# pomelyu/gaussian_splatting_lightning

Measured on AMD Instinct MI355X. Metric: rasterizer fwd+bwd ms & Gaussians·pixels/s @ 1M gauss, 1080p; 1/2/4/8-GPU, higher is better.
Workload: dtype f32; 1 GPU; BASELINE config 3/4: 1M Gaussians, 1920x1080, SH deg 3, fwd+bwd, one view per GPU; gaussians=1000000, width=1920, height=1080, sh_degree=3, parallelism=dp1 (one view per GPU, gradient exchange: none), instances_per_view=4156425, sum_n_contrib=318481376, stage_events=none

## Files before the change

gaussian_splatting_lightning_amd/csrc/gsr_bin.hip:

```cpp
#include <algorithm>

#include "gsr_kernels.h"

namespace gsr {



template <int BKW>
__device__ void bk_instance_offsets(const BucketParams &p, uint32_t g_lo, uint32_t g_hi, uint32_t *s_tmp) {
    const int tid = threadIdx.x, w = tid >> 6, lane = tid & 63;
    uint32_t acc = 0;
    for (uint32_t k = tid; k < g_lo / 256; k += 64 * BKW) acc += p.block_sums[k];
#pragma unroll
    for (int o = 32; o > 0; o >>= 1) acc += (uint32_t)__shfl_xor((int)acc, o);
    if (lane == 0) s_tmp[w] = acc;
    __syncthreads();
    uint32_t base = 0;
    for (int k = 0; k < BKW; k++) base += s_tmp[k];
    __syncthreads();
    for (uint32_t r0 = g_lo; r0 < g_hi; r0 += 4 * 64 * BKW) {
        const uint32_t g = r0 + 4 * (uint32_t)tid;
        uint32_t v[4], loc = 0;
#pragma unroll
        for (int k = 0; k < 4; k++) {
            v[k] = g + k < g_hi ? p.tiles[g + k] : 0u;
            loc += v[k];
        }
        const uint32_t inc = wave_inclusive_scan(loc, lane);
        if (lane == 63) s_tmp[w] = inc;
        __syncthreads();
        uint32_t run = base + inc - loc, all = 0;
        for (int k = 0; k < BKW; k++) {
            if (k < w) run += s_tmp[k];
            all += s_tmp[k];
        }
#pragma unroll
        for (int k = 0; k < 4; k++) {
            if (g + k < g_hi) p.inst_start[g + k] = run;
            run += v[k];
        }
        base += all;
        __syncthreads();
    }
    if (g_hi == p.P && tid == 0) p.inst_start[p.P] = base;
}

__device__ __forceinline__ uint32_t bk_walk_blocks(const BucketParams &p) {
    const uint32_t nbig = *p.nbig;
    return nbig > p.nr ? min(p.nb, nbig) : p.nr;
}

template <bool SCATTER, int BKW>
__global__ __launch_bounds__(64 * BKW) void bk_walk_kernel(BucketParams p) {
    extern __shared__ uint32_t s_tab[];
    __shared__ uint4 s_rec[BKW][64];
    __shared__ uint4 s_aux[BKW][64];
    __shared__ int s_own[BKW][64];
    static_assert(BKW * 64 >= LPT_HIST_WORDS, "the LPT workgroup's histogram lives in s_own");
    const int tid = threadIdx.x, w = tid >> 6, lane = tid & 63;
    const uint32_t b = blockIdx.x, T = p.T, gx = (uint32_t)p.gx;
    if (SCATTER && b == p.nb) {
        constexpr bool xok = 64 * BKW == 1024 && sizeof(s_rec) >= 4 * (LPT_BCNT_WORDS + LPT_XCD + 17);
        lpt_order_block(p.ranges, nullptr, 0, (int)T, p.lpt_shift, p.order, reinterpret_cast<uint32_t *>(&s_own[0][0]),
                        xok ? p.order_xcd : nullptr, reinterpret_cast<uint32_t *>(&s_rec[0][0]), p.gx,
                        (int)((T + gx - 1) / gx), 4);
        return;
    }
    const uint32_t nbw = bk_walk_blocks(p);
    if (b >= nbw) return;
    const bool reg = SCATTER && p.keys_reg != nullptr;
    if (SCATTER && reg) {
        const uint32_t *hrow = p.hist_pre + (size_t)b * T;
        const uint32_t nr = (T + BK_REGION - 1) / BK_REGION;
        for (uint32_t r = tid; r < nr; r += 64 * BKW) {
            const uint32_t t0 = r * BK_REGION;
            uint32_t acc = p.tile_start[t0], v[BK_REGION];
#pragma unroll
            for (int q = 0; q < BK_REGION; q++) v[q] = hrow[min(t0 + q, T - 1)];
#pragma unroll
            for (int q = 0; q < BK_REGION; q++) acc += t0 + q < T ? v[q] : 0u;
            s_tab[r] = acc;
        }
    } else if (SCATTER) {
        const uint32_t *hrow = p.hist_pre + (size_t)b * T;
        for (uint32_t t = tid; t < T; t += 64 * BKW) s_tab[t] = p.tile_start[t] + hrow[t];
    } else {
        for (uint32_t t = tid; t < T; t += 64 * BKW) s_tab[t] = 0u;
    }
    s_own[w][lane] = -1;
    const uint32_t g_lo = min(p.P, b * p.gper), g_hi = min(p.P, g_lo + p.gper);
    if (!SCATTER && b < p.nr) bk_instance_offsets<BKW>(p, g_lo, g_hi, reinterpret_cast<uint32_t *>(&s_aux[0][0]));
    __syncthreads();
    uint32_t g = g_lo + (uint32_t)w * 64 + lane;
    uint32_t n_kept = 0, n_u = 0, n_dep = 0;
    uint4 n_e = make_uint4(0, 0, 0, 0);
    if (g < g_hi) {
        n_kept = p.tiles[g];
        n_e = p.exp_rec[g];
        if (SCATTER) {
            n_u = p.inst_start[g];
            n_dep = p.depth_key[g];
        }
    }
    for (uint32_t g0 = g_lo + (uint32_t)w * 64; g0 < g_hi; g0 += 64 * BKW) {
        const uint32_t kept = n_kept, u = n_u, dep = n_dep;
        const uint4 e = n_e;
        g = g0 + 64 * BKW + lane;
        n_kept = 0;
        if (g < g_hi) {
            n_kept = p.tiles[g];
            n_e = p.exp_rec[g];
            if (SCATTER) {
                n_u = p.inst_start[g];
                n_dep = p.depth_key[g];
            }
        }
        uint32_t len = 0;
        const uint64_t m = (uint64_t)e.x | ((uint64_t)e.y << 32);
        if (kept > 0 && kept <= BIG_GAUSSIAN_TILES) len = m ? 64u - (uint32_t)__builtin_clzll(m) : kept;
        const uint32_t incl = wave_inclusive_scan(len, lane);
        const uint32_t total = (uint32_t)__builtin_amdgcn_readlane((int)incl, 63);
        const uint32_t start = incl - len;
        s_rec[w][lane] = e;
        s_aux[w][lane] = make_uint4(start, u, dep, __float_as_uint(len ? 1.0f / (float)e.w : 0.f));
        int carry = -1;
        for (uint32_t B = 0; B < total; B += 64) {
            const bool marks = len > 0 && start >= B && start < B + 64;
            if (marks) s_own[w][start - B] = lane;
            wave_lds_sync();
            const int o = max(wave_inclusive_max(s_own[w][lane]), carry);
            carry = __builtin_amdgcn_readlane(o, 63);
            wave_lds_sync();
            if (marks) s_own[w][start - B] = -1;
            const uint32_t j = B + (uint32_t)lane;
            if (j < total) {
                const uint4 r = s_rec[w][o];
                const uint4 x = s_aux[w][o];
                const uint32_t c = j - x.x;
                const uint64_t mo = (uint64_t)r.x | ((uint64_t)r.y << 32);
                if (!mo || ((mo >> c) & 1ull)) {
                    const uint32_t tile = rect_tile(c, r.z & 0xffffu, r.z >> 16, r.w, __uint_as_float(x.w), gx);
                    if (!SCATTER) {
                        atomicAdd(&s_tab[tile], 1u);
                    } else {
                        const uint32_t ui = x.y + (mo ? (uint32_t)__popcll(mo & ((1ull << c) - 1ull)) : c);
                        const unsigned long long key = ((unsigned long long)x.z << 32) | ui;
                        if (reg) {
                            const uint32_t slot = atomicAdd(&s_tab[tile / BK_REGION], 1u);
                            p.keys_reg[slot] = key | ((unsigned long long)(tile % BK_REGION) << BK_REG_SHIFT);
                        } else {
                            p.keys[atomicAdd(&s_tab[tile], 1u)] = key;
                        }
                        p.inst_gid[ui] = g0 + (uint32_t)o;
                        p.inv[ui] = INV_NONE;
                    }
                }
            }
        }
        wave_lds_sync();
    }
    const uint32_t nbig = *p.nbig;
    for (uint32_t bi = b; bi < nbig; bi += nbw) {
        const uint32_t gb = p.big_list[bi];
        const uint4 e = p.exp_rec[gb];
        const uint32_t area = p.tiles[gb];
        const float inv_w = 1.0f / (float)e.w;
        const uint32_t u0 = SCATTER ? p.inst_start[gb] : 0u;
        const unsigned long long dk = SCATTER ? ((unsigned long long)p.depth_key[gb] << 32) : 0ull;
        for (uint32_t c = tid; c < area; c += 64 * BKW) {
            const uint32_t tile = rect_tile(c, e.z & 0xffffu, e.z >> 16, e.w, inv_w, gx);
            if (!SCATTER) {
                atomicAdd(&s_tab[tile], 1u);
            } else {
                if (reg) {
                    const uint32_t slot = atomicAdd(&s_tab[tile / BK_REGION], 1u);
                    p.keys_reg[slot] = (dk | (u0 + c)) | ((unsigned long long)(tile % BK_REGION) << BK_REG_SHIFT);
                } else {
                    p.keys[atomicAdd(&s_tab[tile], 1u)] = dk | (u0 + c);
                }
                p.inst_gid[u0 + c] = gb;
                p.inv[u0 + c] = INV_NONE;
            }
        }
    }
    if (!SCATTER) {
        __syncthreads();
        uint32_t *row = p.hist + (size_t)b * T;
        for (uint32_t t = tid; t < T; t += 64 * BKW) row[t] = s_tab[t];
    }
}

__device__ __forceinline__ uint32_t bk_row_block(uint32_t r, uint32_t nb, int xcd_major) {
    if (!xcd_major) return r;
    const uint32_t q = nb >> 3, rem = nb & 7u;
    const uint32_t big = rem * (q + 1);
    uint32_t x, k;
    if (r < big) {
        x = r / (q + 1);
        k = r - x * (q + 1);
    } else {
        const uint32_t r2 = r - big;
        x = rem + r2 / q;
        k = r2 - (x - rem) * q;
    }
    return k * 8 + x;
}

template <int CW, int TW = 64>
__global__ __launch_bounds__(64 * CW) void bk_columns_kernel(BucketParams p) {
    static_assert(TW == 64 || TW == 32, "tiles per workgroup");
    constexpr int NH = 64 / TW;
    __shared__ uint32_t s_sum[CW][64];
    __shared__ uint32_t s_bid;
    __shared__ unsigned long long s_excl;
    const uint32_t *__restrict__ hist = p.hist;
    uint32_t *__restrict__ hist_pre = p.hist_pre;
    const uint32_t nb = bk_walk_blocks(p), T = p.T;
    const int tid = threadIdx.x, w = tid >> 6, lane = tid & 63;
    const int sub = lane % TW, h = lane / TW;
    if (tid == 0) s_bid = atomicAdd(p.ticket, 1u);
    if (blockIdx.x == 0 && p.lpt_bcnt)
        for (uint32_t k = (uint32_t)tid; k < LPT_BCNT_WORDS; k += blockDim.x) p.lpt_bcnt[k] = 0u;
    __syncthreads();
    const uint32_t bid = s_bid;
    const uint32_t t = bid * TW + sub;
    const uint32_t q = (nb + CW - 1) / CW, r0w = min(nb, w * q), r1w = min(nb, r0w + q);
    const uint32_t qh = (q + NH - 1) / NH, r0 = min(r1w, r0w + h * qh), r1 = min(r1w, r0 + qh);
    uint32_t sum = 0;
    const int xm = p.xcd_major;
    if (t < T) {
        uint32_t r = r0;
        for (; r + 8 <= r1; r += 8) {
            uint32_t v[8];
#pragma unroll
            for (int i = 0; i < 8; i++) v[i] = hist[(size_t)bk_row_block(r + i, nb, xm) * T + t];
#pragma unroll
            for (int i = 0; i < 8; i++) sum += v[i];
        }
        for (; r < r1; r++) sum += hist[(size_t)bk_row_block(r, nb, xm) * T + t];
    }
    uint32_t lowsum = 0;
    if constexpr (NH == 2) {
        const uint32_t other = (uint32_t)__shfl_xor((int)sum, 32);
        lowsum = h ? other : 0u;
        sum += other;
    }
    if (h == 0) s_sum[w][sub] = sum;
    __syncthreads();
    uint32_t tot = 0;
#pragma unroll
    for (int i = 0; i < CW; i++) tot += s_sum[i][sub];
    if (w == 0) {
        const uint32_t tv = h == 0 ? tot : 0u;
        const uint32_t inc = wave_inclusive_scan(tv, lane);
        auto agg_of = [&](uint32_t qq) -> uint64_t {
            const uint32_t tq = qq * TW + sub;
            uint64_t v = 0;
            if (tq < T && h == 0)
                for (uint32_t r = 0; r < nb; r++) v += hist[(size_t)r * T + tq];
            return wave_sum_u64(v);
        };
        const uint64_t excl = wave_lookback(p.tile_status, bid, (uint64_t)__builtin_amdgcn_readlane((int)inc, 63),
                                            lane, p.err, p.lb_patience, p.lb_force != 0, agg_of);
        const bool mine = t < T && h == 0;
        if (mine) {
            const uint32_t st = (uint32_t)(excl + inc - tot);
            p.tile_start[t] = st;
            p.ranges[t] = tot ? make_uint2(st, st + tot) : make_uint2(0, 0);
            p.tile_next[t] = st;
            if (t % BK_REGION == 0) p.reg_start[t / BK_REGION] = st;
            p.tile_last[t] = 0u;
            p.tile_loaded[t] = 0u;
            if (t == T - 1) {
                p.tile_start[T] = st + tot;
                p.reg_start[(T + BK_REGION - 1) / BK_REGION] = st + tot;
            }
        }
        const bool l0 = mine && tot > SEG_CAP && tot <= SEG_BLOCK_CAP, l1 = mine && tot > SEG_BLOCK_CAP;
        const uint64_t m0 = __ballot(l0), m1 = __ballot(l1);
        uint32_t b0 = 0, b1 = 0;
        if (lane == 0) {
            if (m0) b0 = atomicAdd(&p.long_cnt[0], (uint32_t)__popcll(m0));
            if (m1) b1 = atomicAdd(&p.long_cnt[1], (uint32_t)__popcll(m1));
        }
        b0 = __builtin_amdgcn_readfirstlane(b0);
        b1 = __builtin_amdgcn_readfirstlane(b1);
        const uint64_t lt = lanemask_lt(lane);
        if (l0) p.long_list[b0 + __popcll(m0 & lt)] = t;
        if (l1) p.long_list[(T + 1) + b1 + __popcll(m1 & lt)] = t;
    }
    uint32_t run = lowsum;
    for (int i = 0; i < w; i++) run += s_sum[i][sub];
    if (t < T) {
        uint32_t r = r0;
        for (; r + 8 <= r1; r += 8) {
            uint32_t v[8];
            size_t row[8];
#pragma unroll
            for (int i = 0; i < 8; i++) {
                row[i] = (size_t)bk_row_block(r + i, nb, xm) * T + t;
                v[i] = hist[row[i]];
            }
#pragma unroll
            for (int i = 0; i < 8; i++) {
                hist_pre[row[i]] = run;
                run += v[i];
            }
        }
        for (; r < r1; r++) {
            const size_t row = (size_t)bk_row_block(r, nb, xm) * T + t;
            const uint32_t v = hist[row];
            hist_pre[row] = run;
            run += v;
        }
    }
}

#ifndef GSR_PART_THREADS
#define GSR_PART_THREADS 256
#endif
#ifndef GSR_PART_ITEMS
#define GSR_PART_ITEMS 4
#endif
constexpr int PART_THREADS = GSR_PART_THREADS;
constexpr int PART_ITEMS = GSR_PART_ITEMS;
constexpr uint32_t PART_CHUNK = PART_THREADS * PART_ITEMS;
#ifndef GSR_PART_MAXR
#define GSR_PART_MAXR 4
#endif
constexpr uint32_t PART_MAXR = GSR_PART_MAXR;
constexpr uint32_t PART_BINS = PART_MAXR * BK_REGION;
static_assert(PART_BINS % 64 == 0 && PART_BINS >= 64, "the bin scan gives each lane of one wave PART_BINS / 64 bins");
__device__ __forceinline__ uint32_t bk_region_of(const uint32_t *rs, uint32_t lo, uint32_t n, uint32_t i) {
    uint32_t hi = n - 1;
    while (lo < hi) {
        const uint32_t mid = (lo + hi + 1) >> 1;
        if (rs[mid] <= i) lo = mid; else hi = mid - 1;
    }
    return lo;
}
__global__ __launch_bounds__(PART_THREADS) void bk_partition_kernel(BucketParams p) {
    __shared__ unsigned long long s_keys[PART_CHUNK];
    __shared__ uint16_t s_bin[PART_CHUNK];
    __shared__ uint32_t s_cnt[PART_BINS], s_lstart[PART_BINS], s_gbase[PART_BINS];
    __shared__ uint32_t s_rstart[PART_MAXR + 1];
    __shared__ uint32_t s_nle[2];
    constexpr unsigned long long TB_MASK = (unsigned long long)(BK_REGION - 1) << BK_REG_SHIFT;
    const uint32_t T = p.T, nr = (T + BK_REGION - 1) / BK_REGION, R = p.tile_start[T];
    const uint32_t c0 = blockIdx.x * PART_CHUNK;
    if (c0 >= R) return;
    const uint32_t n = min(PART_CHUNK, R - c0);
    const int tid = threadIdx.x;
    unsigned long long k[PART_ITEMS];
#pragma unroll
    for (int q = 0; q < PART_ITEMS; q++)
        k[q] = p.keys_reg[c0 + min((uint32_t)(q * PART_THREADS + tid), n - 1)];
    if (tid < 64) {
        const uint32_t rlo = wave_last_le(p.reg_start, nr - 1, c0, tid);
        const uint32_t rhi = wave_last_le(p.reg_start, nr - 1, c0 + n - 1, tid);
        if (tid == 0) {
            s_nle[0] = rlo;
            s_nle[1] = rhi;
        }
    }
    __syncthreads();
    const uint32_t rlo = s_nle[0], nreg = s_nle[1] - rlo + 1;
    if (nreg > PART_MAXR) {
        for (uint32_t i = c0 + tid; i < c0 + n; i += PART_THREADS) {
            const unsigned long long k = p.keys_reg[i];
            const uint32_t t = bk_region_of(p.reg_start, rlo, rlo + nreg, i) * BK_REGION +
                               (uint32_t)((k & TB_MASK) >> BK_REG_SHIFT);
            p.keys[atomicAdd(&p.tile_next[t], 1u)] = k & ~TB_MASK;
        }
        return;
    }
    for (uint32_t j = tid; j <= nreg; j += PART_THREADS) s_rstart[j] = p.reg_start[rlo + j];
    for (uint32_t j = tid; j < nreg * BK_REGION; j += PART_THREADS) s_cnt[j] = 0u;
    __syncthreads();
    uint32_t bin[PART_ITEMS], rank[PART_ITEMS];
#pragma unroll
    for (int q = 0; q < PART_ITEMS; q++) {
        const uint32_t i = (uint32_t)(q * PART_THREADS + tid);
        rank[q] = 0xffffffffu;
        bin[q] = 0;
        if (i < n) {
            uint32_t j = 0;
#pragma unroll
            for (uint32_t step = PART_MAXR / 2; step; step >>= 1)
                if (j + step < nreg && s_rstart[j + step] <= c0 + i) j += step;
            bin[q] = j * BK_REGION + (uint32_t)((k[q] & TB_MASK) >> BK_REG_SHIFT);
            rank[q] = atomicAdd(&s_cnt[bin[q]], 1u);
        }
    }
    __syncthreads();
    const uint32_t nbins = nreg * BK_REGION;
    if (tid < 64) {
        constexpr int PER = PART_BINS / 64;
        uint32_t c[PER], sum = 0;
#pragma unroll
        for (int q = 0; q < PER; q++) {
            const uint32_t b = (uint32_t)(tid * PER + q);
            c[q] = b < nbins ? s_cnt[b] : 0u;
            sum += c[q];
        }
        uint32_t run = wave_inclusive_scan(sum, tid) - sum;
#pragma unroll
        for (int q = 0; q < PER; q++) {
            const uint32_t b = (uint32_t)(tid * PER + q);
            if (b < nbins) {
                s_lstart[b] = run;
                if (c[q]) s_gbase[b] = atomicAdd(&p.tile_next[(rlo + b / BK_REGION) * BK_REGION + b % BK_REGION], c[q]);
            }
            run += c[q];
        }
    }
    __syncthreads();
#pragma unroll
    for (int q = 0; q < PART_ITEMS; q++)
        if (rank[q] != 0xffffffffu) {
            const uint32_t pos = s_lstart[bin[q]] + rank[q];
            s_keys[pos] = k[q] & ~TB_MASK;
            s_bin[pos] = (uint16_t)bin[q];
        }
    __syncthreads();
#pragma unroll
    for (int q = 0; q < PART_ITEMS; q++) {
        const uint32_t i = (uint32_t)(q * PART_THREADS + tid);
        if (i < n) {
            const uint32_t b = s_bin[i];
            p.keys[s_gbase[b] + (i - s_lstart[b])] = s_keys[i];
        }
    }
}

template <int E>
__device__ __forceinline__ void seg_sort_wave32(const unsigned long long *__restrict__ keys, uint32_t start, uint32_t n,
                                                unsigned long long *__restrict__ scratch, int lane,
                                                unsigned long long (&out)[E]) {
    constexpr int LOGE = (E >= 8) ? 3 : (E >= 4) ? 2 : (E >= 2) ? 1 : 0;
    constexpr int IDXB = LOGE + 6;
    const uint32_t base = (uint32_t)lane * E;
    unsigned long long x64[E];
    uint32_t dmin = 0xffffffffu, dmax = 0u;
#pragma unroll
    for (int r = 0; r < E; r++) x64[r] = keys[start + min(base + r, n - 1)];
#pragma unroll
    for (int r = 0; r < E; r++) {
        const bool valid = base + r < n;
        x64[r] = valid ? x64[r] : ~0ull;
        scratch[base + r] = x64[r];
        const uint32_t d = (uint32_t)(x64[r] >> 32);
        if (valid) {
            dmin = min(dmin, d);
            dmax = max(dmax, d);
        }
    }
#pragma unroll
    for (int o = 32; o > 0; o >>= 1) {
        dmin = min(dmin, (uint32_t)__shfl_xor((int)dmin, o));
        dmax = max(dmax, (uint32_t)__shfl_xor((int)dmax, o));
    }
    const uint32_t range = dmax - dmin;
    const int bits = range ? 32 - __builtin_clz(range) : 0;
    const int sh = bits > 32 - IDXB ? bits - (32 - IDXB) : 0;
    uint32_t x[E];
#pragma unroll
    for (int r = 0; r < E; r++)
        x[r] = (base + r < n) ? ((((uint32_t)(x64[r] >> 32) - dmin) >> sh) << IDXB) | (base + r) : 0xffffffffu;
#pragma unroll
    for (int lk = 1; lk < LOGE; lk++) {
#pragma unroll
        for (int lj = lk - 1; lj >= 0; lj--) {
#pragma unroll
            for (int r = 0; r < E; r++) {
                if (r & (1 << lj)) continue;
                const uint32_t a = x[r], c = x[r | (1 << lj)];
                const uint32_t lo = min(a, c), hi = max(a, c);
                const bool asc = (r & (1 << lk)) == 0;
                x[r] = asc ? lo : hi;
                x[r | (1 << lj)] = asc ? hi : lo;
            }
        }
    }
    for (int lk = LOGE > 1 ? LOGE : 1; lk <= LOGE + 6; lk++) {
        const uint32_t flip = (base & (1u << lk)) ? 0xffffffffu : 0u;
#pragma unroll
        for (int r = 0; r < E; r++) x[r] ^= flip;
        for (int lj = lk - 1; lj >= LOGE; lj--) {
            const int lm = 1 << (lj - LOGE);
            const bool lower = (lane & lm) == 0;
            const int addr = (lane ^ lm) << 2;
            uint32_t y[E];
#pragma unroll
            for (int r = 0; r < E; r++) y[r] = (uint32_t)__builtin_amdgcn_ds_bpermute(addr, (int)x[r]);
#pragma unroll
            for (int r = 0; r < E; r++) x[r] = lower ? min(x[r], y[r]) : max(x[r], y[r]);
        }
#pragma unroll
        for (int lj = LOGE - 1; lj >= 0; lj--) {
#pragma unroll
            for (int r = 0; r < E; r++) {
                if (r & (1 << lj)) continue;
                const uint32_t a = x[r], c = x[r | (1 << lj)];
                x[r] = min(a, c);
                x[r | (1 << lj)] = max(a, c);
            }
        }
#pragma unroll
        for (int r = 0; r < E; r++) x[r] ^= flip;
    }
    const uint32_t next0 = (uint32_t)__shfl_down((int)x[0], 1);
    bool tie = false;
#pragma unroll
    for (int r = 0; r < E; r++) {
        const uint32_t nx = r + 1 < E ? x[r + 1] : next0;
        const bool both = base + r + 1 < n && (r + 1 < E || lane < 63);
        tie |= both && (x[r] >> IDXB) == (nx >> IDXB);
    }
    const bool any_tie = __ballot(tie) != 0;
    wave_lds_sync();
#pragma unroll
    for (int r = 0; r < E; r++) out[r] = scratch[x[r] & ((1u << IDXB) - 1u)];
    if (!any_tie) return;
    for (uint32_t it = 0; it < n; it++) {
        bool sw = false;
        auto ce = [&](unsigned long long &a, unsigned long long &b) {
            const bool s = b < a;
            const unsigned long long lo = s ? b : a, hi = s ? a : b;
            a = lo;
            b = hi;
            sw |= s;
        };
        if (E == 1) {
            const unsigned long long y = __shfl_xor(out[0], 1);
            const bool lower = (lane & 1) == 0;
            const unsigned long long v = lower ? (y < out[0] ? y : out[0]) : (y > out[0] ? y : out[0]);
            sw |= v != out[0];
            out[0] = v;
        } else {
#pragma unroll
            for (int r = 0; r + 1 < E; r += 2) ce(out[r], out[r + 1]);
        }
#pragma unroll
        for (int r = 1; r + 1 < E; r += 2) ce(out[r], out[r + 1]);
        const unsigned long long nx = __shfl_down(out[0], 1), pv = __shfl_up(out[E - 1], 1);
        const bool low_end = E > 1 || (lane & 1), high_end = E > 1 || !(lane & 1);
        if (low_end && lane < 63 && nx < out[E - 1]) {
            out[E - 1] = nx;
            sw = true;
        }
        if (high_end && lane > 0 && out[0] < pv) {
            out[0] = pv;
            sw = true;
        }
        if (!__ballot(sw)) return;
    }
}

template <int E>
__device__ __forceinline__ void seg_sort_wave(const unsigned long long *keys, uint32_t start, uint32_t n,
                                              uint32_t *sorted_u, int lane, unsigned long long *scratch) {
    unsigned long long y[E];
    seg_sort_wave32<E>(keys, start, n, scratch, lane, y);
    const uint32_t base = (uint32_t)lane * E;
#pragma unroll
    for (int r = 0; r < E; r++)
        if (base + r < n) sorted_u[start + base + r] = (uint32_t)y[r];
}
template <int E>
__device__ __forceinline__ void seg_sort_wave_to_lds(const unsigned long long *keys, uint32_t start, uint32_t n,
                                                     unsigned long long *lds_out, int lane) {
    unsigned long long y[E];
    seg_sort_wave32<E>(keys, start, n, lds_out, lane, y);
    wave_lds_sync();
    const uint32_t base = (uint32_t)lane * E;
#pragma unroll
    for (int r = 0; r < E; r++) lds_out[base + r] = y[r];
}

constexpr uint32_t SB_CHUNK = 512;
constexpr uint32_t SB_WAVE_SCRATCH = SEG_BLOCK_CAP / 4;

template <int PER>
__device__ __forceinline__ void seg_merge_ranks(const unsigned long long *__restrict__ s_x, uint32_t n, uint32_t nch,
                                                uint32_t start, uint32_t *__restrict__ sorted_u,
                                                unsigned long long *__restrict__ keys_out) {
    const uint32_t span = nch * SB_CHUNK;
    for (uint32_t e0 = 0; e0 < n; e0 += 256 * PER) {
        unsigned long long key[PER];
        uint32_t pos[PER], own[PER];
#pragma unroll
        for (int i = 0; i < PER; i++) {
            const uint32_t e = e0 + threadIdx.x + 256u * i;
            key[i] = e < n ? s_x[e] : ~0ull;
            pos[i] = e & (SB_CHUNK - 1);
            own[i] = e < n ? (e & ~(SB_CHUNK - 1)) : 0u;
        }
        for (uint32_t d = SB_CHUNK; d < span; d += SB_CHUNK) {
            uint32_t lo[PER], idx[PER];
#pragma unroll
            for (int i = 0; i < PER; i++) {
                lo[i] = own[i] + d;
                if (lo[i] >= span) lo[i] -= span;
                idx[i] = lo[i];
            }
#pragma unroll
            for (uint32_t step = SB_CHUNK / 2; step; step >>= 1) {
#pragma unroll
                for (int i = 0; i < PER; i++)
                    if (s_x[idx[i] + step - 1] < key[i]) idx[i] += step;
            }
#pragma unroll
            for (int i = 0; i < PER; i++)
                pos[i] += idx[i] - lo[i] + (s_x[idx[i]] < key[i] ? 1u : 0u);
        }
#pragma unroll
        for (int i = 0; i < PER; i++) {
            const uint32_t e = e0 + threadIdx.x + 256u * i;
            if (e >= n) continue;
            if (keys_out) keys_out[start + pos[i]] = key[i];
            else sorted_u[start + pos[i]] = (uint32_t)key[i];
        }
    }
}

__device__ __forceinline__ void seg_lds_sort(const unsigned long long *__restrict__ keys, uint32_t start, uint32_t n,
                                             uint32_t *__restrict__ sorted_u, unsigned long long *__restrict__ keys_out,
                                             unsigned long long *__restrict__ s_x, int w, int lane,
                                             uint32_t *t_mid = nullptr) {
    const uint32_t nch = (n + SB_CHUNK - 1) / SB_CHUNK;
    for (uint32_t c = (uint32_t)w; c < nch; c += 4) {
        const uint32_t c0 = c * SB_CHUNK;
        seg_sort_wave_to_lds<8>(keys, start + c0, min(SB_CHUNK, n - c0), s_x + c0, lane);
    }
    __syncthreads();
    if (t_mid) *t_mid = stamp_now();
    if (n <= 256u * 4u) seg_merge_ranks<4>(s_x, n, nch, start, sorted_u, keys_out);
    else seg_merge_ranks<8>(s_x, n, nch, start, sorted_u, keys_out);
    __syncthreads();
}

__device__ void seg_tile_chunked(const SegSortParams &p, uint2 rg, uint32_t n, unsigned long long *s_x, int w,
                                 int lane) {
    for (uint32_t c0 = 0; c0 < n; c0 += SEG_BLOCK_CAP)
        seg_lds_sort(p.keys, rg.x + c0, min(SEG_BLOCK_CAP, n - c0), nullptr, p.keys2, s_x, w, lane);
    __threadfence();
    __syncthreads();
    const unsigned long long *kk = p.keys2 + rg.x;
    const uint32_t nch = (n + SEG_BLOCK_CAP - 1) / SEG_BLOCK_CAP;
    for (uint32_t e = threadIdx.x; e < n; e += 256) {
        const unsigned long long key = kk[e];
        const uint32_t c = e / SEG_BLOCK_CAP;
        uint32_t pos = e - c * SEG_BLOCK_CAP;
        for (uint32_t c2 = 0; c2 < nch; c2++) {
            if (c2 == c) continue;
            const unsigned long long *ch = kk + c2 * SEG_BLOCK_CAP;
            uint32_t lo = 0, hi = min(SEG_BLOCK_CAP, n - c2 * SEG_BLOCK_CAP);
            while (lo < hi) {
                const uint32_t mid = (lo + hi) >> 1;
                if (ch[mid] < key) lo = mid + 1; else hi = mid;
            }
            pos += lo;
        }
        p.sorted_u[rg.x + pos] = (uint32_t)key;
    }
    __syncthreads();
}

__global__ __launch_bounds__(256, 6) void seg_sort_kernel(SegSortParams p) {
    __shared__ unsigned long long s_x[SEG_BLOCK_CAP];
    const int lane = threadIdx.x & 63, w = threadIdx.x >> 6;
    const uint32_t n0 = p.long_cnt[0], nlong = n0 + p.long_cnt[1];
    for (uint32_t i = blockIdx.x; i < nlong; i += gridDim.x) {
        const uint32_t tile = p.tile_order ? p.tile_order[i] : i < n0 ? p.long_list[i] : p.long_list[p.T + 1 + (i - n0)];
        const uint2 rg = p.ranges[tile];
        const uint32_t n = rg.y - rg.x;
        if (n <= SEG_CAP) continue;
        if (n > SEG_BLOCK_CAP) {
            seg_tile_chunked(p, rg, n, s_x, w, lane);
            continue;
        }
        const uint32_t t0 = p.stamps ? stamp_now() : 0u;
        uint32_t t1 = 0;
        seg_lds_sort(p.keys, rg.x, n, p.sorted_u, nullptr, s_x, w, lane, p.stamps ? &t1 : nullptr);
        if (p.stamps && threadIdx.x == 0 && i < (uint32_t)STAMP_SLOTS) p.stamps[i] = make_uint4(t0, t1, stamp_now(), n);
    }
    const uint32_t s0 = p.tile_order ? nlong : 0u;
    for (uint32_t j = s0 + blockIdx.x * 4 + (uint32_t)w; j < p.T; j += gridDim.x * 4) {
        const uint32_t tile = p.tile_order ? p.tile_order[j] : j;
        const uint2 rg = p.ranges[tile];
        const uint32_t n = rg.y - rg.x;
        if (n == 0 || n > SEG_CAP) continue;
        unsigned long long *scratch = s_x + w * SB_WAVE_SCRATCH;
        if (n <= 64u) seg_sort_wave<1>(p.keys, rg.x, n, p.sorted_u, lane, scratch);
        else if (n <= 128u) seg_sort_wave<2>(p.keys, rg.x, n, p.sorted_u, lane, scratch);
        else if (n <= 256u) seg_sort_wave<4>(p.keys, rg.x, n, p.sorted_u, lane, scratch);
        else seg_sort_wave<8>(p.keys, rg.x, n, p.sorted_u, lane, scratch);
    }
}

template <bool SCATTER>
static void launch_walk(hipStream_t s, const BucketParams &p, uint32_t grid) {
    const size_t lds = sizeof(uint32_t) * p.T;
    if (lds + 40 * 1024 <= 160 * 1024) {
        if (lds > 65536)
            (void)hipFuncSetAttribute(reinterpret_cast<const void *>(&bk_walk_kernel<SCATTER, 16>),
                                      hipFuncAttributeMaxDynamicSharedMemorySize, (int)lds);
        bk_walk_kernel<SCATTER, 16><<<grid, 64 * 16, lds, s>>>(p);
    } else {
        if (lds > 65536)
            (void)hipFuncSetAttribute(reinterpret_cast<const void *>(&bk_walk_kernel<SCATTER, 8>),
                                      hipFuncAttributeMaxDynamicSharedMemorySize, (int)lds);
        bk_walk_kernel<SCATTER, 8><<<grid, 64 * 8, lds, s>>>(p);
    }
}

void launch_bucket_count(hipStream_t s, const BucketParams &p) {
    launch_walk<false>(s, p, p.nb);
    bk_columns_kernel<16, 32><<<div_up(p.T, 32), 1024, 0, s>>>(p);
}

void launch_bucket_scatter(hipStream_t s, const BucketParams &p) {
    launch_walk<true>(s, p, p.nb + (p.order ? 1u : 0u));
    if (p.keys_reg) bk_partition_kernel<<<div_up(p.R, PART_CHUNK), PART_THREADS, 0, s>>>(p);
}

void launch_seg_sort(hipStream_t s, const SegSortParams &p0) {
    if (p0.T == 0) return;
    SegSortParams p = p0;
    p.stamps = tuning(K_stamp) ? stamp_buffer(2) : nullptr;
    seg_sort_kernel<<<std::min(div_up(p.T, 4), 4096u), 256, 0, s>>>(p);
}

}
```

Baseline: 2757000 billion Gaussians·pixels/s.

## Tune segmented sort: strided wave loads, 6-item merge path, uniform stamp checks

Segmented per-tile sort changes: the wave sort now loads keys with a lane-strided pattern (64*r+lane), giving coalesced global reads and conflict-free scratch writes in place of contiguous per-lane chunks. A 6-items-per-thread merge-rank variant is added for mid-sized tiles to reduce idle work, and the stamp pointer check and wave index are forced into scalar registers to keep control flow uniform. The merge's bounds check now uses the sentinel key instead of a recomputed index. This risks correctness if the bitonic network assumed contiguous index layout, and it adds another template instantiation.

```diff
diff --git a/gaussian_splatting_lightning_amd/csrc/gsr_bin.hip b/gaussian_splatting_lightning_amd/csrc/gsr_bin.hip
--- a/gaussian_splatting_lightning_amd/csrc/gsr_bin.hip
+++ b/gaussian_splatting_lightning_amd/csrc/gsr_bin.hip
@@ -439,16 +439,18 @@
                                                 unsigned long long (&out)[E]) {
     constexpr int LOGE = (E >= 8) ? 3 : (E >= 4) ? 2 : (E >= 2) ? 1 : 0;
     constexpr int IDXB = LOGE + 6;
+    asm volatile("" : "+v"(lane));
     const uint32_t base = (uint32_t)lane * E;
     unsigned long long x64[E];
     uint32_t dmin = 0xffffffffu, dmax = 0u;
-#pragma unroll
-    for (int r = 0; r < E; r++) x64[r] = keys[start + min(base + r, n - 1)];
+    auto src = [&](int r) { return 64u * (uint32_t)r + (uint32_t)lane; };
+#pragma unroll
+    for (int r = 0; r < E; r++) x64[r] = keys[start + min(src(r), n - 1)];
 #pragma unroll
     for (int r = 0; r < E; r++) {
-        const bool valid = base + r < n;
+        const bool valid = src(r) < n;
         x64[r] = valid ? x64[r] : ~0ull;
-        scratch[base + r] = x64[r];
+        scratch[src(r)] = x64[r];
         const uint32_t d = (uint32_t)(x64[r] >> 32);
         if (valid) {
             dmin = min(dmin, d);
@@ -466,7 +468,7 @@
     uint32_t x[E];
 #pragma unroll
     for (int r = 0; r < E; r++)
-        x[r] = (base + r < n) ? ((((uint32_t)(x64[r] >> 32) - dmin) >> sh) << IDXB) | (base + r) : 0xffffffffu;
+        x[r] = (src(r) < n) ? ((((uint32_t)(x64[r] >> 32) - dmin) >> sh) << IDXB) | src(r) : 0xffffffffu;
 #pragma unroll
     for (int lk = 1; lk < LOGE; lk++) {
 #pragma unroll
@@ -616,28 +618,36 @@
         }
 #pragma unroll
         for (int i = 0; i < PER; i++) {
-            const uint32_t e = e0 + threadIdx.x + 256u * i;
-            if (e >= n) continue;
+            if (key[i] == ~0ull) continue;
             if (keys_out) keys_out[start + pos[i]] = key[i];
             else sorted_u[start + pos[i]] = (uint32_t)key[i];
         }
     }
 }
 
-__device__ __forceinline__ void seg_lds_sort(const unsigned long long *__restrict__ keys, uint32_t start, uint32_t n,
-                                             uint32_t *__restrict__ sorted_u, unsigned long long *__restrict__ keys_out,
-                                             unsigned long long *__restrict__ s_x, int w, int lane,
-                                             uint32_t *t_mid = nullptr) {
+__device__ __forceinline__ bool seg_stamps_on(const uint4 *stamps) {
+    unsigned long long v = (unsigned long long)stamps;
+    asm volatile("" : "+s"(v));
+    return v != 0;
+}
+
+__device__ __forceinline__ uint32_t seg_lds_sort(const unsigned long long *__restrict__ keys, uint32_t start, uint32_t n,
+                                                 uint32_t *__restrict__ sorted_u,
+                                                 unsigned long long *__restrict__ keys_out,
+                                                 unsigned long long *__restrict__ s_x, int w, int lane,
+                                                 const uint4 *stamps = nullptr) {
     const uint32_t nch = (n + SB_CHUNK - 1) / SB_CHUNK;
     for (uint32_t c = (uint32_t)w; c < nch; c += 4) {
         const uint32_t c0 = c * SB_CHUNK;
         seg_sort_wave_to_lds<8>(keys, start + c0, min(SB_CHUNK, n - c0), s_x + c0, lane);
     }
     __syncthreads();
-    if (t_mid) *t_mid = stamp_now();
+    const uint32_t t_mid = seg_stamps_on(stamps) ? stamp_now() : 0u;
     if (n <= 256u * 4u) seg_merge_ranks<4>(s_x, n, nch, start, sorted_u, keys_out);
+    else if (n <= 256u * 6u) seg_merge_ranks<6>(s_x, n, nch, start, sorted_u, keys_out);
     else seg_merge_ranks<8>(s_x, n, nch, start, sorted_u, keys_out);
     __syncthreads();
+    return t_mid;
 }
 
 __device__ void seg_tile_chunked(const SegSortParams &p, uint2 rg, uint32_t n, unsigned long long *s_x, int w,
@@ -669,7 +679,7 @@
 
 __global__ __launch_bounds__(256, 6) void seg_sort_kernel(SegSortParams p) {
     __shared__ unsigned long long s_x[SEG_BLOCK_CAP];
-    const int lane = threadIdx.x & 63, w = threadIdx.x >> 6;
+    const int lane = threadIdx.x & 63, w = __builtin_amdgcn_readfirstlane((int)(threadIdx.x >> 6));
     const uint32_t n0 = p.long_cnt[0], nlong = n0 + p.long_cnt[1];
     for (uint32_t i = blockIdx.x; i < nlong; i += gridDim.x) {
         const uint32_t tile = p.tile_order ? p.tile_order[i] : i < n0 ? p.long_list[i] : p.long_list[p.T + 1 + (i - n0)];
@@ -680,10 +690,10 @@
             seg_tile_chunked(p, rg, n, s_x, w, lane);
             continue;
         }
-        const uint32_t t0 = p.stamps ? stamp_now() : 0u;
-        uint32_t t1 = 0;
-        seg_lds_sort(p.keys, rg.x, n, p.sorted_u, nullptr, s_x, w, lane, p.stamps ? &t1 : nullptr);
-        if (p.stamps && threadIdx.x == 0 && i < (uint32_t)STAMP_SLOTS) p.stamps[i] = make_uint4(t0, t1, stamp_now(), n);
+        const uint32_t t0 = seg_stamps_on(p.stamps) ? stamp_now() : 0u;
+        const uint32_t t1 = seg_lds_sort(p.keys, rg.x, n, p.sorted_u, nullptr, s_x, w, lane, p.stamps);
+        if (seg_stamps_on(p.stamps) && threadIdx.x == 0 && i < (uint32_t)STAMP_SLOTS)
+            p.stamps[i] = make_uint4(t0, t1, stamp_now(), n);
     }
     const uint32_t s0 = p.tile_order ? nlong : 0u;
     for (uint32_t j = s0 + blockIdx.x * 4 + (uint32_t)w; j < p.T; j += gridDim.x * 4) {
```

New measurement: 2775000 billion Gaussians·pixels/s, median of 6. About the same (+0.7%).
